# weidafeng/Efficient-SlowFast

Measured on AMD Instinct MI355X. Metric: clips/sec (8x8 224^2 SlowFast-R50+CMDA, train step fwd+bwd+allreduce+SGD), higher is better.
Workload: dtype f32

## Files before the change

### efficient-slowfast_amd/csrc/backward.hip

```cpp
#include "common.h"
#include <stdlib.h>

namespace {

constexpr int TPB = 256;


inline int pow2ceil_b(int v) {
  int p = 1;
  while (p < v) p <<= 1;
  return p;
}

template <int VEC>
__device__ __forceinline__ void bn_g(const float* __restrict__ dy, int dy_cs, int dy_coff,
                                     const float* __restrict__ y, int y_cs, int y_coff, long r, long THW, int HW,
                                     int rep, int relu, int c, float (&g)[VEC]) {
  long r0 = r;
  if (rep > 1) {
    const long n = r / THW, rem = r - n * THW;
    const long t = rem / HW, hw = rem - t * HW;
    r0 = (n * (THW / HW) * rep + t * rep) * HW + hw;
  }
#pragma unroll
  for (int e = 0; e < VEC; ++e) g[e] = 0.f;
  for (int q = 0; q < rep; ++q) {
    const float* d = dy + (r0 + (long)q * HW) * dy_cs + dy_coff + c;
    if (VEC == 4) {
      const f32x4 v = *reinterpret_cast<const f32x4*>(d);
#pragma unroll
      for (int e = 0; e < 4; ++e) g[e] += v[e];
    } else {
      g[0] += d[0];
    }
  }
  if (relu == 3) {
    if (VEC == 4) {
      const unsigned mk = reinterpret_cast<const unsigned char*>(y)[r0 * y_cs + (c >> 2)];
#pragma unroll
      for (int e = 0; e < 4; ++e)
        if (!((mk >> e) & 1u)) g[e] = 0.f;
    }
  } else if (relu) {
    const float* yp = y + r0 * y_cs + y_coff + c;
    if (VEC == 4) {
      const f32x4 v = *reinterpret_cast<const f32x4*>(yp);
#pragma unroll
      for (int e = 0; e < 4; ++e)
        if (!(v[e] > 0.f) || (relu == 2 && !(v[e] < 6.f))) g[e] = 0.f;
    } else if (!(yp[0] > 0.f) || (relu == 2 && !(yp[0] < 6.f))) {
      g[0] = 0.f;
    }
  }
}

template <int VEC>
__global__ void bn_bwd_partial_kernel(const float* __restrict__ dy, int dy_cs, int dy_coff,
                                      const float* __restrict__ y, int y_cs, int y_coff,
                                      const float* __restrict__ z, int z_cs, int z_coff, long group_rows, int chunks,
                                      int S, long THW, int HW, int C, int rep, int relu,
                                      const float* __restrict__ mean, const float* __restrict__ invstd, int CB,
                                      float* __restrict__ partial, unsigned* tickets, float* __restrict__ o1,
                                      float* __restrict__ o2, float* __restrict__ acc1, float* __restrict__ acc2) {
  __shared__ float red[2 * TPB * VEC];
  const int blk = blockIdx.x, cb = blockIdx.y;
  const int cl = threadIdx.x % CB, rl = threadIdx.x / CB, rpi = TPB / CB;
  const int c = (cb * CB + cl) * VEC;
  const int n = blk / chunks, ck = blk - n * chunks;
  const long per = (group_rows + chunks - 1) / chunks;
  const long gend = (long)(n + 1) * group_rows;
  const long r0 = (long)n * group_rows + (long)ck * per;
  const long r1 = (r0 + per < gend) ? r0 + per : gend;
  const int so = (n % S) * C;
  float s1[VEC], s2[VEC];
#pragma unroll
  for (int e = 0; e < VEC; ++e) { s1[e] = 0.f; s2[e] = 0.f; }
  if (c < C) {
    float mu[VEC], is[VEC];
#pragma unroll
    for (int e = 0; e < VEC; ++e) { mu[e] = mean[so + c + e]; is[e] = invstd[so + c + e]; }
    long r = r0 + rl;
    if constexpr (VEC == 4) if (rep == 1 && (relu == 0 || relu == 3)) {
      const unsigned char* const mk = reinterpret_cast<const unsigned char*>(y);
      for (; r + 3 * (long)rpi < r1; r += 4 * (long)rpi) {
        f32x4 gv[4], zq[4];
        unsigned mb[4];
#pragma unroll
        for (int u = 0; u < 4; ++u) {
          const long ru = r + (long)u * rpi;
          gv[u] = *reinterpret_cast<const f32x4*>(dy + ru * dy_cs + dy_coff + c);
          zq[u] = *reinterpret_cast<const f32x4*>(z + ru * z_cs + z_coff + c);
          mb[u] = relu == 3 ? mk[ru * y_cs + (c >> 2)] : 0xFu;
        }
#pragma unroll
        for (int u = 0; u < 4; ++u)
#pragma unroll
// ... 15 lines not shown
        zv[0] = z[r * z_cs + z_coff + c];
      }
#pragma unroll
      for (int e = 0; e < VEC; ++e) {
        s1[e] += g[e];
        s2[e] = fmaf(g[e], (zv[e] - mu[e]) * is[e], s2[e]);
      }
    }
  }
#pragma unroll
  for (int e = 0; e < VEC; ++e) {
    red[threadIdx.x * VEC + e] = s1[e];
    red[(TPB + threadIdx.x) * VEC + e] = s2[e];
  }
  __syncthreads();
  if (rl == 0 && c < C) {
#pragma unroll
    for (int e = 0; e < VEC; ++e) {
      float t1 = 0.f, t2 = 0.f;
      for (int i = 0; i < rpi; ++i) {
        t1 += red[(i * CB + cl) * VEC + e];
        t2 += red[(TPB + i * CB + cl) * VEC + e];
      }
      if (tickets) {
        sf_store_sc1(partial + ((long)blk * 2 + 0) * C + c + e, t1);
        sf_store_sc1(partial + ((long)blk * 2 + 1) * C + c + e, t2);
      } else {
        partial[((long)blk * 2 + 0) * C + c + e] = t1;
        partial[((long)blk * 2 + 1) * C + c + e] = t2;
      }
    }
  }
  if (!tickets) return;
  if (!sf_ticket_last(tickets + cb, gridDim.x)) return;
  const int P = gridDim.x;
  const int cbase = cb * CB * VEC;
  const int ncg = (C - cbase) < CB * VEC ? (C - cbase) : CB * VEC;
  const int q = threadIdx.x & 3;
  for (int item = threadIdx.x >> 2; item < S * ncg; item += TPB / 4) {
    const int sp = item / ncg, cc = cbase + (item - sp * ncg);
    double a1 = 0.0, a2 = 0.0;
    for (int i = q; i < P; i += 4) {
      if ((i / chunks) % S != sp) continue;
      a1 += (double)partial[((long)i * 2 + 0) * C + cc];
      a2 += (double)partial[((long)i * 2 + 1) * C + cc];
    }
    a1 += __shfl_xor(a1, 1, 64);
    a2 += __shfl_xor(a2, 1, 64);
    a1 += __shfl_xor(a1, 2, 64);
    a2 += __shfl_xor(a2, 2, 64);
    if (q == 0) {
      const int o = sp * C + cc;
      o1[o] = (float)a1;
      o2[o] = (float)a2;
      if (acc1) {
        acc1[o] += (float)a1;
        acc2[o] += (float)a2;
      }
    }
  }
}

__global__ void pair_final_kernel(const float* __restrict__ partial, int C, int P, int chunks, int S,
                                  float* __restrict__ o1, float* __restrict__ o2, float* __restrict__ acc1,
                                  float* __restrict__ acc2) {
  __shared__ double r1[64], r2[64];
  const int o = blockIdx.x;
  const int sp = o / C, c = o - sp * C;
  double s1 = 0.0, s2 = 0.0;
  int i = threadIdx.x;
  if (S == 1) {
    double a1[4] = {0.0, 0.0, 0.0, 0.0}, a2[4] = {0.0, 0.0, 0.0, 0.0};
    for (; i + 192 < P; i += 256) {
      float t1[4], t2[4];
#pragma unroll
      for (int u = 0; u < 4; ++u) {
        t1[u] = partial[((long)(i + 64 * u) * 2 + 0) * C + c];
        t2[u] = partial[((long)(i + 64 * u) * 2 + 1) * C + c];
      }
#pragma unroll
      for (int u = 0; u < 4; ++u) {
        a1[u] += (double)t1[u];
        a2[u] += (double)t2[u];
      }
    }
    s1 = (a1[0] + a1[1]) + (a1[2] + a1[3]);
    s2 = (a2[0] + a2[1]) + (a2[2] + a2[3]);
  }
  for (; i < P; i += 64) {
    if ((i / chunks) % S != sp) continue;
    s1 += (double)partial[((long)i * 2 + 0) * C + c];
    s2 += (double)partial[((long)i * 2 + 1) * C + c];
  }
// ... 257 lines not shown
  const int c = (int)(idx % C);
  const long r = idx / C;
  const float v = alpha * a[r * a_cs + a_coff + c];
  float* o = out + r * out_cs + out_coff + c;
  *o = accumulate ? *o + v : v;
}

__global__ void act_bwd_kernel(const float* __restrict__ dy, int dy_cs, int dy_coff, const float* __restrict__ y,
                               int y_cs, int y_coff, int act, float* __restrict__ dx, int dx_cs, int dx_coff, int C,
                               int accumulate, long total) {
  const long idx = (long)blockIdx.x * TPB + threadIdx.x;
  if (idx >= total) return;
  const int c = (int)(idx % C);
  const long r = idx / C;
  const float yv = y[r * y_cs + y_coff + c];
  const bool pass = (yv > 0.f) && (act != SF_ACT_RELU6 || yv < 6.f);
  const float v = pass ? dy[r * dy_cs + dy_coff + c] : 0.f;
  float* o = dx + r * dx_cs + dx_coff + c;
  *o = accumulate ? *o + v : v;
}

}

constexpr int MAX_P = 1024;
static inline void red_geometry(long rows, int C, int vec, int* CB, int* P) {
  const int cv = sf_cdiv(C, vec);
  *CB = pow2ceil_b(cv) < TPB ? pow2ceil_b(cv) : TPB;
  const int rpi = TPB / *CB;
  long p = rows / ((long)rpi * 8);
  if (p < 1) p = 1;
  if (p > MAX_P) p = MAX_P;
  *P = (int)p;
}
extern "C" long sf_bn_bwd_ws_floats(int C) { return (long)MAX_P * 2 * C; }

static int bn_bwd_reduce_launch(const float* dy, int dy_cs, int dy_coff, const float* y, int y_cs, int y_coff,
                                const float* z, int z_cs, int z_coff, int N, int T, int H, int W, int C, int S,
                                int rep, int relu, const float* mean, const float* invstd, float* dbeta,
                                float* dgamma, float* ws, void* stream, float* dbeta_acc = nullptr,
                                float* dgamma_acc = nullptr) {
  if ((dbeta_acc == nullptr) != (dgamma_acc == nullptr)) return SF_EINVAL;
  if (!dy || !z || !mean || !invstd || !dbeta || !dgamma || !ws || (relu && !y)) return SF_EINVAL;
  if (relu == 3 && (rep != 1 || (C % 4) != 0 || y_cs != C / 4 || y_coff != 0)) return SF_EINVAL;
  if (N <= 0 || T <= 0 || H <= 0 || W <= 0 || C <= 0 || rep <= 0 || S <= 0 || N % S != 0) return SF_EINVAL;
  if (S > 1 && N > MAX_P) return SF_EINVAL;
  const long rows = (long)N * T * H * W;
  const bool vec4 = (C % 4 == 0) && (dy_cs % 4 == 0) && (dy_coff % 4 == 0) && (z_cs % 4 == 0) && (z_coff % 4 == 0) &&
                    sf_aligned16(dy) && sf_aligned16(z) &&
                    (!relu || relu == 3 || ((y_cs % 4 == 0) && (y_coff % 4 == 0) && sf_aligned16(y)));
  if (relu == 3 && !vec4) return SF_EINVAL;
  const int groups = S > 1 ? N : 1;
  const long group_rows = rows / groups;
  int CB, P;
  const bool ring = sf_ticket_ring_ready((hipStream_t)stream);
  red_geometry(group_rows, C, vec4 ? 4 : 1, &CB, &P);
  const bool small = ring && S == 1 && P <= 16;
  const bool few = !small && ring && S == 1 && vec4 && C >= 256;
  const bool fused = few || small;
  const int max_p = few ? 64 : (small ? 512 : MAX_P);
  if (few && CB > 16) {
    CB = 16;
    long pp = group_rows / ((long)(TPB / CB) * 8);
    P = (int)(pp < 1 ? 1 : (pp > max_p ? max_p : pp));
  }
  if (P > max_p) P = max_p;
  if ((long)P * groups > max_p) P = max_p / groups;
  if (P < 1) return SF_EINVAL;
  const int chunks = P;
  P = chunks * groups;
  const int ncb = sf_cdiv(sf_cdiv(C, vec4 ? 4 : 1), CB);
  unsigned* tickets = fused ? sf_ticket_slots(ncb) : nullptr;
  if (fused && !tickets) return SF_ELAUNCH;
  if (vec4)
    hipLaunchKernelGGL(bn_bwd_partial_kernel<4>, dim3(P, ncb), dim3(TPB), 0, (hipStream_t)stream, dy, dy_cs, dy_coff,
                       y, y_cs, y_coff, z, z_cs, z_coff, group_rows, chunks, S, (long)T * H * W, H * W, C, rep, relu,
                       mean, invstd, CB, ws, tickets, dbeta, dgamma, dbeta_acc, dgamma_acc);
  else
    hipLaunchKernelGGL(bn_bwd_partial_kernel<1>, dim3(P, ncb), dim3(TPB), 0, (hipStream_t)stream, dy, dy_cs, dy_coff,
                       y, y_cs, y_coff, z, z_cs, z_coff, group_rows, chunks, S, (long)T * H * W, H * W, C, rep, relu,
                       mean, invstd, CB, ws, tickets, dbeta, dgamma, dbeta_acc, dgamma_acc);
  if (!fused)
    hipLaunchKernelGGL(pair_final_kernel, dim3(S * C), dim3(64), 0, (hipStream_t)stream, ws, C, P, chunks, S, dbeta,
                       dgamma, dbeta_acc, dgamma_acc);
  SF_CHECK_LAUNCH();
  return SF_OK;
}

extern "C" int sf_bn_bwd_reduce(const float* dy, int dy_cs, int dy_coff, const float* y, int y_cs, int y_coff,
                                const float* z, int z_cs, int z_coff, int N, int T, int H, int W, int C, int rep,
                                int relu, const float* mean, const float* invstd, float* dbeta, float* dgamma,
                                float* ws, void* stream) {
  return bn_bwd_reduce_launch(dy, dy_cs, dy_coff, y, y_cs, y_coff, z, z_cs, z_coff, N, T, H, W, C, 1, rep, relu, mean,
                              invstd, dbeta, dgamma, ws, stream);
}

extern "C" int sf_bn_bwd_reduce_acc(const float* dy, int dy_cs, int dy_coff, const float* y, int y_cs, int y_coff,
                                    const float* z, int z_cs, int z_coff, int N, int T, int H, int W, int C, int rep,
                                    int relu, const float* mean, const float* invstd, float* dbeta, float* dgamma,
                                    float* ws, float* dbeta_acc, float* dgamma_acc, void* stream) {
  return bn_bwd_reduce_launch(dy, dy_cs, dy_coff, y, y_cs, y_coff, z, z_cs, z_coff, N, T, H, W, C, 1, rep, relu, mean,
                              invstd, dbeta, dgamma, ws, stream, dbeta_acc, dgamma_acc);
}

extern "C" int sf_bn_bwd_reduce_split(const float* dy, int dy_cs, int dy_coff, const float* y, int y_cs, int y_coff,
                                      const float* z, int z_cs, int z_coff, int N, int T, int H, int W, int C,
                                      int nsplit, int rep, int relu, const float* mean, const float* invstd,
                                      float* dbeta, float* dgamma, float* ws, void* stream) {
  return bn_bwd_reduce_launch(dy, dy_cs, dy_coff, y, y_cs, y_coff, z, z_cs, z_coff, N, T, H, W, C, nsplit, rep, relu,
                              mean, invstd, dbeta, dgamma, ws, stream);
}

static int bn_bwd_apply_launch(const float* dy, int dy_cs, int dy_coff, const float* y, int y_cs, int y_coff,
                               const float* z, int z_cs, int z_coff, int N, int T, int H, int W, int C, int S, int rep,
                               int relu, const float* mean, const float* invstd, const float* gamma,
                               const float* dbeta, const float* dgamma, float* dz, int dz_cs, int dz_coff,
                               float* dres, int dres_cs, int dres_coff, int dres_acc, void* stream) {
// ... 589 lines not shown
```

### efficient-slowfast_amd/csrc/common.h

```cpp
#pragma once
#include <hip/hip_runtime.h>
#include <stdint.h>
#include "sfhip.h"

typedef float f32x2 __attribute__((ext_vector_type(2)));
typedef float f32x4 __attribute__((ext_vector_type(4)));
typedef float f32x16 __attribute__((ext_vector_type(16)));

#define SF_CHECK_LAUNCH()                                   \
  do {                                                      \
    if (hipPeekAtLastError() != hipSuccess) return SF_ELAUNCH; \
  } while (0)

__device__ __forceinline__ int xcd_remap(int b, int n) {
  const int q = n >> 3, r = n & 7, x = b & 7, i = b >> 3;
  return (x < r ? x * (q + 1) : r * (q + 1) + (x - r) * q) + i;
}

__device__ __forceinline__ float sf_act(float v, int act) {
  if (act == SF_ACT_RELU) return v > 0.f ? v : 0.f;
  if (act == SF_ACT_RELU6) return fminf(fmaxf(v, 0.f), 6.f);
  if (act == SF_ACT_HSIGMOID) return fminf(fmaxf(v + 3.f, 0.f), 6.f) * (1.f / 6.f);
  if (act == SF_ACT_SIGMOID) return 1.f / (1.f + __expf(-v));
  return v;
}

static inline bool sf_aligned16(const void* p) { return (reinterpret_cast<uintptr_t>(p) & 15) == 0; }
static inline int sf_cdiv(long a, long b) { return (int)((a + b - 1) / b); }

constexpr int SF_SWEEP_PARTS_MAX = 8;
int sf_sweep_parts(long units, int tiles);
int sf_attn_nw();

unsigned* sf_ticket_slots(int n);
bool sf_ticket_ring_ready(hipStream_t stream);

struct SfLdsAttr { unsigned long long done = 0; };
static inline bool sf_ensure_dyn_lds(SfLdsAttr& m, const void* fn, int bytes) {
  int dev = 0;
  if (hipGetDevice(&dev) != hipSuccess) return false;
  if (dev >= 0 && dev < 64 && ((m.done >> dev) & 1ull)) return true;
  if (hipFuncSetAttribute(fn, hipFuncAttributeMaxDynamicSharedMemorySize, bytes) != hipSuccess) return false;
  if (dev >= 0 && dev < 64) m.done |= 1ull << dev;
  return true;
}

__device__ __forceinline__ void sf_store_sc1(float* p, float v) {
  __hip_atomic_store(p, v, __ATOMIC_RELAXED, __HIP_MEMORY_SCOPE_AGENT);
}

__device__ __forceinline__ bool sf_ticket_last(unsigned* cnt, unsigned total) {
  __shared__ int s_last;
  asm volatile("s_waitcnt vmcnt(0)" ::: "memory");
  __syncthreads();
  if (threadIdx.x == 0) {
    const unsigned old = __hip_atomic_fetch_add(cnt, 1u, __ATOMIC_RELAXED, __HIP_MEMORY_SCOPE_AGENT);
    const bool last = old == total - 1u;
    if (last) {
      __hip_atomic_store(cnt, 0u, __ATOMIC_RELAXED, __HIP_MEMORY_SCOPE_AGENT);
      __builtin_amdgcn_fence(__ATOMIC_ACQUIRE, "agent");
      asm volatile("s_waitcnt vmcnt(0)" ::: "memory");
    }
    s_last = last ? 1 : 0;
  }
  __syncthreads();
  return s_last != 0;
}
```

### efficient-slowfast_amd/csrc/elementwise.hip

```cpp
#include "common.h"

namespace {

constexpr int TPB = 256;

__global__ void ncthw_to_ndhwc_kernel(const float* __restrict__ src, float* __restrict__ dst, int N, int C,
                                      int T, int H, int W, int cpad, int ph, int pw, int Hp, int Wp, long total) {
  const long idx = (long)blockIdx.x * TPB + threadIdx.x;
  if (idx >= total) return;
  const int wp = (int)(idx % Wp);
  long r = idx / Wp;
  const int hp = (int)(r % Hp);
  r /= Hp;
  const int t = (int)(r % T);
  const int n = (int)(r / T);
  const int h = hp - ph, w = wp - pw;
  const bool in = (unsigned)h < (unsigned)H && (unsigned)w < (unsigned)W;
  float* o = dst + idx * cpad;
  const long plane = (long)T * H * W;
  const float* s = src + ((long)n * C * T + t) * H * W + (long)h * W + w;
  if (cpad == 4) {
    f32x4 v = {0.f, 0.f, 0.f, 0.f};
    if (in) {
      v[0] = s[0];
// ... 336 lines not shown
}

__global__ void copy_channels_kernel(const float* __restrict__ in, int in_cs, int in_coff, float* __restrict__ out,
                                     int out_cs, int out_coff, int out_cmul, int C, long total) {
  const long idx = (long)blockIdx.x * TPB + threadIdx.x;
  if (idx >= total) return;
  const int c = (int)(idx % C);
  const long r = idx / C;
  out[r * out_cs + out_coff + (long)c * out_cmul] = in[r * in_cs + in_coff + c];
}

__global__ void channel_shuffle_kernel(const float* __restrict__ in, int in_cs, int in_coff, float* __restrict__ out,
                                       int out_cs, int out_coff, int G, int C, int accumulate, long total) {
  const long idx = (long)blockIdx.x * TPB + threadIdx.x;
  if (idx >= total) return;
  const int c = (int)(idx % C);
  const long r = idx / C;
  const float v = in[r * in_cs + in_coff + (c % G) * (C / G) + c / G];
  float* const o = out + r * out_cs + out_coff + c;
  *o = accumulate ? *o + v : v;
}


constexpr int STAT_MAX_P = 1024;

struct StatsFinal {
  double inv_rows, unbias;
  float* mean; float* var;
  const float* gamma; const float* beta;
  float eps, momentum;
  float* run_mean; float* run_var;
  float* invstd; float* scale; float* shift;
  unsigned* tickets;
};

__device__ __forceinline__ void stats_finish(const StatsFinal& f, int o, double s1, double s2, float k) {
  const double md = s1 * f.inv_rows;
  double v = s2 * f.inv_rows - md * md;
  if (v < 0.0) v = 0.0;
  const double m = md + (double)k;
  f.mean[o] = (float)m;
  f.var[o] = (float)v;
  if (f.gamma) {
    const float is = (float)(1.0 / sqrt(v + (double)f.eps));
    const float sc = f.gamma[o] * is;
    f.invstd[o] = is;
    f.scale[o] = sc;
    f.shift[o] = f.beta[o] - (float)m * sc;
    if (f.run_mean) {
      f.run_mean[o] = (1.f - f.momentum) * f.run_mean[o] + f.momentum * (float)m;
      f.run_var[o] = (1.f - f.momentum) * f.run_var[o] + f.momentum * (float)(v * f.unbias);
    }
  }
}

template <int VEC>
__global__ void stats_partial_kernel(const float* __restrict__ x, int cs, int coff, long group_rows, int chunks,
                                     int S, int C, int CB, float* __restrict__ partial, const StatsFinal fin) {
  __shared__ float red[2 * TPB * VEC];
  const int blk = blockIdx.x, cb = blockIdx.y;
  const int cl = threadIdx.x % CB, rl = threadIdx.x / CB, rpi = TPB / CB;
  const int c = (cb * CB + cl) * VEC;
  const int n = blk / chunks, ck = blk - n * chunks;
  const long per = (group_rows + chunks - 1) / chunks;
  const long gend = (long)(n + 1) * group_rows;
  const long r0 = (long)n * group_rows + (long)ck * per;
  const long r1 = (r0 + per < gend) ? r0 + per : gend;
  const long krow = (long)(n % S) * group_rows;
  float s1[VEC], s2[VEC], k[VEC];
#pragma unroll
  for (int e = 0; e < VEC; ++e) { s1[e] = 0.f; s2[e] = 0.f; k[e] = 0.f; }
  if (c < C) {
#pragma unroll
    for (int e = 0; e < VEC; ++e) k[e] = x[krow * cs + coff + c + e];
    long r = r0 + rl;
    if constexpr (VEC == 4) {
      for (; r + 3 * (long)rpi < r1; r += 4 * (long)rpi) {
        f32x4 v[4];
#pragma unroll
        for (int u = 0; u < 4; ++u) v[u] = *reinterpret_cast<const f32x4*>(x + (r + (long)u * rpi) * cs + coff + c);
#pragma unroll
        for (int u = 0; u < 4; ++u)
#pragma unroll
          for (int e = 0; e < 4; ++e) {
            const float d = v[u][e] - k[e];
            s1[e] += d;
            s2[e] = fmaf(d, d, s2[e]);
          }
// ... 9 lines not shown
          s2[e] = fmaf(d, d, s2[e]);
        }
      } else {
        const float d = x[r * cs + coff + c] - k[0];
        s1[0] += d;
        s2[0] = fmaf(d, d, s2[0]);
      }
    }
  }
#pragma unroll
  for (int e = 0; e < VEC; ++e) {
    red[threadIdx.x * VEC + e] = s1[e];
    red[(TPB + threadIdx.x) * VEC + e] = s2[e];
  }
  __syncthreads();
  if (rl == 0 && c < C) {
#pragma unroll
    for (int e = 0; e < VEC; ++e) {
      float t1 = 0.f, t2 = 0.f;
      for (int i = 0; i < rpi; ++i) {
        t1 += red[(i * CB + cl) * VEC + e];
        t2 += red[(TPB + i * CB + cl) * VEC + e];
      }
      if (fin.tickets) {
        sf_store_sc1(partial + ((long)blk * 2 + 0) * C + c + e, t1);
        sf_store_sc1(partial + ((long)blk * 2 + 1) * C + c + e, t2);
      } else {
        partial[((long)blk * 2 + 0) * C + c + e] = t1;
        partial[((long)blk * 2 + 1) * C + c + e] = t2;
      }
    }
  }
  if (!fin.tickets) return;
  if (!sf_ticket_last(fin.tickets + cb, gridDim.x)) return;
  const int P = gridDim.x;
  const int cbase = cb * CB * VEC;
  const int ncg = (C - cbase) < CB * VEC ? (C - cbase) : CB * VEC;
  const int q = threadIdx.x & 3;
  for (int item = threadIdx.x >> 2; item < S * ncg; item += TPB / 4) {
    const int sp = item / ncg, cc = cbase + (item - sp * ncg);
    double s1 = 0.0, s2 = 0.0;
    for (int i = q; i < P; i += 4) {
      if ((i / chunks) % S != sp) continue;
      s1 += (double)partial[((long)i * 2 + 0) * C + cc];
      s2 += (double)partial[((long)i * 2 + 1) * C + cc];
    }
    s1 += __shfl_xor(s1, 1, 64);
    s2 += __shfl_xor(s2, 1, 64);
    s1 += __shfl_xor(s1, 2, 64);
    s2 += __shfl_xor(s2, 2, 64);
    if (q == 0) stats_finish(fin, sp * C + cc, s1, s2, x[(long)sp * group_rows * cs + coff + cc]);
  }
}

__global__ void stats_final_kernel(const float* __restrict__ x, int cs, int coff, long group_rows, int chunks, int S,
                                   const float* __restrict__ partial, int C, int P, double inv_rows, double unbias,
                                   float* __restrict__ mean, float* __restrict__ var,
                                   const float* __restrict__ gamma, const float* __restrict__ beta, float eps,
                                   float momentum, float* __restrict__ run_mean, float* __restrict__ run_var,
                                   float* __restrict__ invstd, float* __restrict__ scale, float* __restrict__ shift) {
  __shared__ double r1[64], r2[64];
  const int o = blockIdx.x;
  const int sp = o / C, c = o - sp * C;
  double s1 = 0.0, s2 = 0.0;
  int i = threadIdx.x;
  if (S == 1) {
    double a1[4] = {0.0, 0.0, 0.0, 0.0}, a2[4] = {0.0, 0.0, 0.0, 0.0};
    for (; i + 192 < P; i += 256) {
      float t1[4], t2[4];
#pragma unroll
      for (int u = 0; u < 4; ++u) {
        t1[u] = partial[((long)(i + 64 * u) * 2 + 0) * C + c];
        t2[u] = partial[((long)(i + 64 * u) * 2 + 1) * C + c];
      }
#pragma unroll
      for (int u = 0; u < 4; ++u) {
        a1[u] += (double)t1[u];
        a2[u] += (double)t2[u];
      }
    }
    s1 = (a1[0] + a1[1]) + (a1[2] + a1[3]);
    s2 = (a2[0] + a2[1]) + (a2[2] + a2[3]);
  }
  for (; i < P; i += 64) {
    if ((i / chunks) % S != sp) continue;
// ... 200 lines not shown
    __syncthreads();
    if (co < (unsigned)it.Cout && c0 + lx < (unsigned)it.cin_pad)
      for (unsigned tap = 0; tap < taps; ++tap)
        it.wp[((long)co * taps + tap) * it.cin_pad + c0 + lx] = seg[ly * pitch + lx * taps + tap];
    return;
  }
  const unsigned Q = (unsigned)it.Cin * (unsigned)it.taps;
  const unsigned tq = (Q + 31u) / 32u;
  const unsigned t = b - nbw;
  const unsigned tco = t / tq, tqi = t - tco * tq;
  const unsigned q0 = tqi * 32u, co0 = tco * 32u;
  const unsigned lx = threadIdx.x & 31u, ly = threadIdx.x >> 5;
#pragma unroll
  for (int k = 0; k < 4; ++k) {
    const unsigned co = co0 + ly + 8u * k, q = q0 + lx;
    tile[ly + 8 * k][lx] = (co < (unsigned)it.Cout && q < Q) ? it.w[(long)co * Q + q] : 0.f;
  }
  __syncthreads();
#pragma unroll
  for (int k = 0; k < 4; ++k) {
    const unsigned q = q0 + ly + 8u * k, co = co0 + lx;
    if (q < Q && co < (unsigned)it.cout_pad) it.wtp[(long)q * it.cout_pad + co] = tile[lx][ly + 8 * k];
  }
}

inline int pow2ceil(int v) {
  int p = 1;
  while (p < v) p <<= 1;
  return p;
}

}

#include <atomic>
namespace {
constexpr int TICKET_RING = 1 << 16, TICKET_MAXDEV = 16;
unsigned* g_ticket_ring[TICKET_MAXDEV] = {};
std::atomic<unsigned> g_ticket_next[TICKET_MAXDEV];
}

bool sf_ticket_ring_ready(hipStream_t stream) {
  int dev = 0;
  if (hipGetDevice(&dev) != hipSuccess || dev < 0 || dev >= TICKET_MAXDEV) return false;
  if (g_ticket_ring[dev]) return true;
  hipStreamCaptureStatus st = hipStreamCaptureStatusNone;
  if (hipStreamIsCapturing(stream, &st) != hipSuccess || st != hipStreamCaptureStatusNone) return false;
  unsigned* p = nullptr;
  if (hipMalloc(&p, TICKET_RING * sizeof(unsigned)) != hipSuccess) return false;
  if (hipMemset(p, 0, TICKET_RING * sizeof(unsigned)) != hipSuccess) return false;
  g_ticket_ring[dev] = p;
  return true;
}

unsigned* sf_ticket_slots(int n) {
  int dev = 0;
  if (hipGetDevice(&dev) != hipSuccess || dev < 0 || dev >= TICKET_MAXDEV || n <= 0 || n > 4096) return nullptr;
  if (!g_ticket_ring[dev]) return nullptr;
  const unsigned take = ((unsigned)n + 63u) & ~63u;
  unsigned off;
  do {
    off = g_ticket_next[dev].fetch_add(take) % TICKET_RING;
  } while (off + take > (unsigned)TICKET_RING);
  return g_ticket_ring[dev] + off;
}

extern "C" int sf_abi_version(void) { return 1; }
extern "C" const char* sf_build_arch(void) { return "gfx950"; }

extern "C" int sf_ncthw_to_ndhwc(const float* src, float* dst, int N, int C, int T, int H, int W, int cpad,
                                 int ph, int pw, int Wp, void* stream) {
  if (!src || !dst || N <= 0 || C <= 0 || T <= 0 || H <= 0 || W <= 0 || cpad < C || ph < 0 || pw < 0 ||
      Wp < W + 2 * pw)
    return SF_EINVAL;
  if (cpad == 4 && !sf_aligned16(dst)) return SF_EALIGN;
  const int Hp = H + 2 * ph;
  const long total = (long)N * T * Hp * Wp;
  hipLaunchKernelGGL(ncthw_to_ndhwc_kernel, dim3(sf_cdiv(total, TPB)), dim3(TPB), 0, (hipStream_t)stream, src,
                     dst, N, C, T, H, W, cpad, ph, pw, Hp, Wp, total);
  SF_CHECK_LAUNCH();
  return SF_OK;
}

extern "C" int sf_ndhwc_to_ncthw(const float* src, int cs, int coff, float* dst, int N, int C, int T, int H,
                                 int W, void* stream) {
  if (!src || !dst || N <= 0 || C <= 0 || T <= 0 || H <= 0 || W <= 0 || cs < coff + C) return SF_EINVAL;
  const long thw = (long)T * H * W;
  const long total = (long)N * C * thw;
  hipLaunchKernelGGL(ndhwc_to_ncthw_kernel, dim3(sf_cdiv(total, TPB)), dim3(TPB), 0, (hipStream_t)stream, src,
                     cs, coff, dst, C, thw, total);
  SF_CHECK_LAUNCH();
  return SF_OK;
}

extern "C" int sf_pool_fwd(const sf_pool_desc* d, const float* in, float* out, void* stream) {
  if (!d || !in || !out || d->C <= 0 || d->kT <= 0 || d->kH <= 0 || d->kW <= 0) return SF_EINVAL;
  if (d->N <= 0 || d->To <= 0 || d->Ho <= 0 || d->Wo <= 0) return SF_EINVAL;
// ... 78 lines not shown
  hipLaunchKernelGGL(tmax_partial_kernel, dim3(POOL_P, ncb, N), dim3(TPB), 0, (hipStream_t)stream, x, cs, coff, T,
                     H * W, C, alpha, CB, ws);
  const float inv = 1.f / (float)((long)(T / alpha) * H * W);
  hipLaunchKernelGGL(tmax_final_kernel, dim3(sf_cdiv(C, TPB), N), dim3(TPB), 0, (hipStream_t)stream, ws, C, inv,
                     pooled);
  SF_CHECK_LAUNCH();
  return SF_OK;
}

extern "C" int sf_gate_apply(const float* x, int cs, int coff, int N, int T, int H, int W, int C, int alpha,
                             const float* pooled, const float* w3, const float* scale, const float* bias, int act,
                             float* out, int out_cs, int out_coff, void* stream) {
  if (!x || !pooled || !out || N <= 0 || C <= 0 || alpha <= 0 || (T % alpha) != 0) return SF_EINVAL;
  if ((scale == nullptr) != (bias == nullptr)) return SF_EINVAL;
  if (act != SF_ACT_NONE && act != SF_ACT_RELU) return SF_EINVAL;
  const bool vec4 = (C % 4 == 0) && (cs % 4 == 0) && (coff % 4 == 0) && (out_cs % 4 == 0) && (out_coff % 4 == 0) &&
                    sf_aligned16(x) && sf_aligned16(out);
  const long rows = (long)(T / alpha) * H * W;
  const long total = rows * (vec4 ? C / 4 : C);
  int gx = sf_cdiv(total, TPB);
  if (gx > 2048) gx = 2048;
  const size_t shm = (size_t)C * sizeof(float);
  if (vec4)
    hipLaunchKernelGGL(gate_apply_kernel<4>, dim3(gx, N), dim3(TPB), shm, (hipStream_t)stream, x, cs, coff, T,
                       H * W, C, alpha, pooled, w3, scale, bias, act, out, out_cs, out_coff);
  else
    hipLaunchKernelGGL(gate_apply_kernel<1>, dim3(gx, N), dim3(TPB), shm, (hipStream_t)stream, x, cs, coff, T,
                       H * W, C, alpha, pooled, w3, scale, bias, act, out, out_cs, out_coff);
  SF_CHECK_LAUNCH();
  return SF_OK;
}


extern "C" long sf_channel_stats_ws_floats(int C) { return (long)STAT_MAX_P * 2 * C; }

static int stats_launch(const float* x, int cs, int coff, int groups, long group_rows, int S, int C, float* mean,
                        float* var, float* ws, const float* gamma, const float* beta, float eps, float momentum,
                        float* run_mean, float* run_var, float* invstd, float* scale, float* shift, hipStream_t s) {
  if (groups > STAT_MAX_P || S <= 0 || groups % S != 0) return SF_EINVAL;
  const bool vec4 = (C % 4 == 0) && (cs % 4 == 0) && (coff % 4 == 0) && sf_aligned16(x);
  const int cv = sf_cdiv(C, vec4 ? 4 : 1);
  const bool ring = sf_ticket_ring_ready(s);
  const int CB = pow2ceil(cv) < TPB ? pow2ceil(cv) : TPB;
  const bool fused = ring && S == 1 && groups == 1 && group_rows / ((long)(TPB / CB) * 8) <= 16;
  const int rpi = TPB / CB;
  const int max_p = fused ? 512 : STAT_MAX_P;
  if (groups > max_p) return SF_EINVAL;
  long ch = group_rows / ((long)rpi * 8);
  if (ch < 1) ch = 1;
  if (ch * groups > max_p) ch = max_p / groups;
  const int chunks = (int)ch, P = chunks * groups;
  const long srows = group_rows * (groups / S);
  const int ncb = sf_cdiv(cv, CB);
  StatsFinal fin;
  fin.inv_rows = 1.0 / (double)srows;
  fin.unbias = srows > 1 ? (double)srows / (double)(srows - 1) : 1.0;
  fin.mean = mean; fin.var = var; fin.gamma = gamma; fin.beta = beta; fin.eps = eps; fin.momentum = momentum;
  fin.run_mean = run_mean; fin.run_var = run_var; fin.invstd = invstd; fin.scale = scale; fin.shift = shift;
  fin.tickets = fused ? sf_ticket_slots(ncb) : nullptr;
  if (fused && !fin.tickets) return SF_ELAUNCH;
  if (vec4)
    hipLaunchKernelGGL(stats_partial_kernel<4>, dim3(P, ncb), dim3(TPB), 0, s, x, cs, coff, group_rows, chunks, S, C, CB,
                       ws, fin);
  else
    hipLaunchKernelGGL(stats_partial_kernel<1>, dim3(P, ncb), dim3(TPB), 0, s, x, cs, coff, group_rows, chunks, S, C, CB,
                       ws, fin);
  if (!fused)
    hipLaunchKernelGGL(stats_final_kernel, dim3(S * C), dim3(64), 0, s, x, cs, coff, group_rows, chunks, S, ws, C, P,
                       fin.inv_rows, fin.unbias, mean, var, gamma, beta, eps, momentum, run_mean, run_var, invstd, scale,
                       shift);
  SF_CHECK_LAUNCH();
  return SF_OK;
}

__global__ void stats_merge_kernel(const float* __restrict__ parts, int P, int C, const StatsFinal f) {
  __shared__ double red[16][9];
  const int quad = blockIdx.x, nq = C >> 2;
  const int tid = threadIdx.x, lane = tid & 63, wave = tid >> 6, nwave = blockDim.x >> 6;
  const f32x4 R = *reinterpret_cast<const f32x4*>(parts + (long)quad * 16 + 4);
  double n = 0.0, s1[4] = {0.0, 0.0, 0.0, 0.0}, s2[4] = {0.0, 0.0, 0.0, 0.0};
  auto add = [&](const f32x4& cnt, const f32x4& k, const f32x4& a1, const f32x4& a2) {
    const double ni = (double)cnt[0];
    n += ni;
#pragma unroll
    for (int e = 0; e < 4; ++e) {
      const double dk = (double)k[e] - (double)R[e], t1 = (double)a1[e];
      s1[e] += t1 + ni * dk;
      s2[e] += (double)a2[e] + dk * (2.0 * t1 + ni * dk);
    }
  };
  const int step = blockDim.x;
  int i = tid;
  for (; i + 3 * step < P; i += 4 * step) {
    f32x4 v[4][4];
#pragma unroll
    for (int u = 0; u < 4; ++u) {
      const float* q = parts + ((long)(i + u * step) * nq + quad) * 16;
#pragma unroll
      for (int w = 0; w < 4; ++w) v[u][w] = *reinterpret_cast<const f32x4*>(q + 4 * w);
    }
#pragma unroll
    for (int u = 0; u < 4; ++u) add(v[u][0], v[u][1], v[u][2], v[u][3]);
  }
// ... 8 lines not shown
#pragma unroll
    for (int e = 0; e < 4; ++e) {
      s1[e] += __shfl_xor(s1[e], off, 64);
      s2[e] += __shfl_xor(s2[e], off, 64);
    }
  }
  if (lane == 0) {
    red[wave][0] = n;
#pragma unroll
    for (int e = 0; e < 4; ++e) { red[wave][1 + e] = s1[e]; red[wave][5 + e] = s2[e]; }
  }
  __syncthreads();
  if (tid < 4) {
    double N = 0.0, t1 = 0.0, t2 = 0.0;
    for (int w = 0; w < nwave; ++w) { N += red[w][0]; t1 += red[w][1 + tid]; t2 += red[w][5 + tid]; }
    StatsFinal g = f;
    g.inv_rows = 1.0 / N;
    g.unbias = N > 1.0 ? N / (N - 1.0) : 1.0;
    stats_finish(g, quad * 4 + tid, t1, t2, R[tid]);
  }
}

extern "C" int sf_bn_train_stats_merge(const float* parts, int P, int C, const float* gamma, const float* beta, float eps,
                                       float momentum, float* run_mean, float* run_var, float* mean, float* var,
                                       float* invstd, float* scale, float* shift, void* stream) {
  if (!parts || P <= 0 || C <= 0 || (C % 4) != 0 || !gamma || !beta || !mean || !var || !invstd || !scale || !shift)
    return SF_EINVAL;
  if ((run_mean == nullptr) != (run_var == nullptr) || !sf_aligned16(parts)) return SF_EINVAL;
  StatsFinal fin;
  fin.inv_rows = 1.0; fin.unbias = 1.0;
  fin.mean = mean; fin.var = var; fin.gamma = gamma; fin.beta = beta; fin.eps = eps; fin.momentum = momentum;
  fin.run_mean = run_mean; fin.run_var = run_var; fin.invstd = invstd; fin.scale = scale; fin.shift = shift;
  fin.tickets = nullptr;
  hipLaunchKernelGGL(stats_merge_kernel, dim3(C / 4), dim3(P > 1024 ? 1024 : 256), 0, (hipStream_t)stream, parts, P, C,
                     fin);
  SF_CHECK_LAUNCH();
  return SF_OK;
}

extern "C" int sf_channel_stats(const float* x, int cs, int coff, long rows, int C, float* mean, float* var,
                                float* ws, void* stream) {
  if (!x || !mean || !var || !ws || rows <= 0 || C <= 0) return SF_EINVAL;
  return stats_launch(x, cs, coff, 1, rows, 1, C, mean, var, ws, nullptr, nullptr, 0.f, 0.f, nullptr, nullptr, nullptr,
                      nullptr, nullptr, (hipStream_t)stream);
}

extern "C" int sf_bn_train_stats(const float* x, int cs, int coff, long rows, int C, const float* gamma,
                                 const float* beta, float eps, float momentum, float* run_mean, float* run_var,
                                 float* mean, float* var, float* invstd, float* scale, float* shift, float* ws,
                                 void* stream) {
  if (!x || !gamma || !beta || !mean || !var || !invstd || !scale || !shift || !ws || rows <= 0 || C <= 0)
    return SF_EINVAL;
  if ((run_mean == nullptr) != (run_var == nullptr)) return SF_EINVAL;
  return stats_launch(x, cs, coff, 1, rows, 1, C, mean, var, ws, gamma, beta, eps, momentum, run_mean, run_var,
                      invstd, scale, shift, (hipStream_t)stream);
}

extern "C" int sf_bn_train_stats_split(const float* x, int cs, int coff, int N, long rows_per_sample, int C,
                                       int nsplit, const float* gamma, const float* beta, float eps, float momentum,
                                       float* run_mean, float* run_var, float* mean, float* var, float* invstd,
                                       float* scale, float* shift, float* ws, void* stream) {
  if (!x || !gamma || !beta || !mean || !var || !invstd || !scale || !shift || !ws || N <= 0 ||
      rows_per_sample <= 0 || C <= 0 || nsplit <= 0 || N % nsplit != 0)
    return SF_EINVAL;
  if ((run_mean == nullptr) != (run_var == nullptr)) return SF_EINVAL;
  return stats_launch(x, cs, coff, N, rows_per_sample, nsplit, C, mean, var, ws, gamma, beta, eps, momentum, run_mean,
// ... 124 lines not shown
```

Measured before the change: 150.8.

## Use two-level ticketed fold for BN stats and backward channel reductions

For single-group BatchNorm forward stats and backward dbeta/dgamma reductions, the final cross-block reduction now runs in two levels. Groups of 32 partial blocks are summed by the last-arriving block of each group into a double-precision L2 workspace, and the globally last block folds those group sums. New geometry caps channels per block at 64 so more column blocks and row chunks run in parallel. The ticket allocator is also reworked to work under stream capture, so the fused path is always available, with a fallback final kernel when no ticket slots are granted. This drops the separate final kernel launch and the serial single-block reduction over up to 1024 partials, at the cost of extra atomics, workspace and more complex allocation.

New measurement: 150.5. No clear change (-0.2%).

```diff
diff --git a/efficient-slowfast_amd/csrc/backward.hip b/efficient-slowfast_amd/csrc/backward.hip
--- a/efficient-slowfast_amd/csrc/backward.hip
+++ b/efficient-slowfast_amd/csrc/backward.hip
@@ -54,14 +54,27 @@
   }
 }
 
+struct PairFin {
+  float* o1; float* o2; float* acc1; float* acc2;
+  __device__ void operator()(int c, double s1, double s2) const {
+    o1[c] = (float)s1;
+    o2[c] = (float)s2;
+    if (acc1) {
+      acc1[c] += (float)s1;
+      acc2[c] += (float)s2;
+    }
+  }
+};
+
 template <int VEC>
 __global__ void bn_bwd_partial_kernel(const float* __restrict__ dy, int dy_cs, int dy_coff,
                                       const float* __restrict__ y, int y_cs, int y_coff,
                                       const float* __restrict__ z, int z_cs, int z_coff, long group_rows, int chunks,
                                       int S, long THW, int HW, int C, int rep, int relu,
                                       const float* __restrict__ mean, const float* __restrict__ invstd, int CB,
-                                      float* __restrict__ partial, unsigned* tickets, float* __restrict__ o1,
-                                      float* __restrict__ o2, float* __restrict__ acc1, float* __restrict__ acc2) {
+                                      float* __restrict__ partial, double* l2, unsigned* tickets,
+                                      float* __restrict__ o1, float* __restrict__ o2, float* __restrict__ acc1,
+                                      float* __restrict__ acc2) {
   __shared__ float red[2 * TPB * VEC];
   const int blk = blockIdx.x, cb = blockIdx.y;
   const int cl = threadIdx.x % CB, rl = threadIdx.x / CB, rpi = TPB / CB;
@@ -143,33 +156,11 @@
     }
   }
   if (!tickets) return;
-  if (!sf_ticket_last(tickets + cb, gridDim.x)) return;
   const int P = gridDim.x;
   const int cbase = cb * CB * VEC;
   const int ncg = (C - cbase) < CB * VEC ? (C - cbase) : CB * VEC;
-  const int q = threadIdx.x & 3;
-  for (int item = threadIdx.x >> 2; item < S * ncg; item += TPB / 4) {
-    const int sp = item / ncg, cc = cbase + (item - sp * ncg);
-    double a1 = 0.0, a2 = 0.0;
-    for (int i = q; i < P; i += 4) {
-      if ((i / chunks) % S != sp) continue;
-      a1 += (double)partial[((long)i * 2 + 0) * C + cc];
-      a2 += (double)partial[((long)i * 2 + 1) * C + cc];
-    }
-    a1 += __shfl_xor(a1, 1, 64);
-    a2 += __shfl_xor(a2, 1, 64);
-    a1 += __shfl_xor(a1, 2, 64);
-    a2 += __shfl_xor(a2, 2, 64);
-    if (q == 0) {
-      const int o = sp * C + cc;
-      o1[o] = (float)a1;
-      o2[o] = (float)a2;
-      if (acc1) {
-        acc1[o] += (float)a1;
-        acc2[o] += (float)a2;
-      }
-    }
-  }
+  sf_fold_finish(partial, l2, tickets + cb * (1 + sf_fold_groups(P)), blk, P, C, cbase, ncg,
+                 PairFin{o1, o2, acc1, acc2});
 }
 
 __global__ void pair_final_kernel(const float* __restrict__ partial, int C, int P, int chunks, int S,
@@ -493,7 +484,10 @@
   if (p > MAX_P) p = MAX_P;
   *P = (int)p;
 }
-extern "C" long sf_bn_bwd_ws_floats(int C) { return (long)MAX_P * 2 * C; }
+extern "C" long sf_bn_bwd_ws_floats(int C) { return (long)MAX_P * 2 * C + 2 + sf_fold_l2_floats(C); }
+static inline double* bwd_ws_l2(float* ws, int C) {
+  return reinterpret_cast<double*>((reinterpret_cast<uintptr_t>(ws + (long)MAX_P * 2 * C) + 7) & ~(uintptr_t)7);
+}
 
 static int bn_bwd_reduce_launch(const float* dy, int dy_cs, int dy_coff, const float* y, int y_cs, int y_coff,
                                 const float* z, int z_cs, int z_coff, int N, int T, int H, int W, int C, int S,
@@ -513,36 +507,43 @@
   const int groups = S > 1 ? N : 1;
   const long group_rows = rows / groups;
   int CB, P;
-  const bool ring = sf_ticket_ring_ready((hipStream_t)stream);
+  if (S == 1) {
+    const int vec = vec4 ? 4 : 1;
+    sf_fold_geometry(rows, sf_cdiv(C, vec), vec, &CB, &P);
+    const int ncb = sf_cdiv(sf_cdiv(C, vec), CB);
+    double* l2 = bwd_ws_l2(ws, C);
+    const long nslots = (long)ncb * (1 + sf_fold_groups(P));
+    unsigned* tickets = nslots <= 4096 ? sf_ticket_slots((int)nslots, (hipStream_t)stream) : nullptr;
+    if (vec4)
+      hipLaunchKernelGGL(bn_bwd_partial_kernel<4>, dim3(P, ncb), dim3(TPB), 0, (hipStream_t)stream, dy, dy_cs, dy_coff,
+                         y, y_cs, y_coff, z, z_cs, z_coff, rows, P, 1, (long)T * H * W, H * W, C, rep, relu, mean, invstd,
+                         CB, ws, l2, tickets, dbeta, dgamma, dbeta_acc, dgamma_acc);
+    else
+      hipLaunchKernelGGL(bn_bwd_partial_kernel<1>, dim3(P, ncb), dim3(TPB), 0, (hipStream_t)stream, dy, dy_cs, dy_coff,
+                         y, y_cs, y_coff, z, z_cs, z_coff, rows, P, 1, (long)T * H * W, H * W, C, rep, relu, mean, invstd,
+                         CB, ws, l2, tickets, dbeta, dgamma, dbeta_acc, dgamma_acc);
+    if (!tickets)
+      hipLaunchKernelGGL(sf_fold_final_kernel<PairFin>, dim3(ncb), dim3(TPB), 0, (hipStream_t)stream, ws, l2, P, C,
+                         CB * vec, PairFin{dbeta, dgamma, dbeta_acc, dgamma_acc});
+    SF_CHECK_LAUNCH();
+    return SF_OK;
+  }
   red_geometry(group_rows, C, vec4 ? 4 : 1, &CB, &P);
-  const bool small = ring && S == 1 && P <= 16;
-  const bool few = !small && ring && S == 1 && vec4 && C >= 256;
-  const bool fused = few || small;
-  const int max_p = few ? 64 : (small ? 512 : MAX_P);
-  if (few && CB > 16) {
-    CB = 16;
-    long pp = group_rows / ((long)(TPB / CB) * 8);
-    P = (int)(pp < 1 ? 1 : (pp > max_p ? max_p : pp));
-  }
-  if (P > max_p) P = max_p;
-  if ((long)P * groups > max_p) P = max_p / groups;
+  if ((long)P * groups > MAX_P) P = MAX_P / groups;
   if (P < 1) return SF_EINVAL;
   const int chunks = P;
   P = chunks * groups;
   const int ncb = sf_cdiv(sf_cdiv(C, vec4 ? 4 : 1), CB);
-  unsigned* tickets = fused ? sf_ticket_slots(ncb) : nullptr;
-  if (fused && !tickets) return SF_ELAUNCH;
   if (vec4)
     hipLaunchKernelGGL(bn_bwd_partial_kernel<4>, dim3(P, ncb), dim3(TPB), 0, (hipStream_t)stream, dy, dy_cs, dy_coff,
                        y, y_cs, y_coff, z, z_cs, z_coff, group_rows, chunks, S, (long)T * H * W, H * W, C, rep, relu,
-                       mean, invstd, CB, ws, tickets, dbeta, dgamma, dbeta_acc, dgamma_acc);
+                       mean, invstd, CB, ws, nullptr, nullptr, dbeta, dgamma, dbeta_acc, dgamma_acc);
   else
     hipLaunchKernelGGL(bn_bwd_partial_kernel<1>, dim3(P, ncb), dim3(TPB), 0, (hipStream_t)stream, dy, dy_cs, dy_coff,
                        y, y_cs, y_coff, z, z_cs, z_coff, group_rows, chunks, S, (long)T * H * W, H * W, C, rep, relu,
-                       mean, invstd, CB, ws, tickets, dbeta, dgamma, dbeta_acc, dgamma_acc);
-  if (!fused)
-    hipLaunchKernelGGL(pair_final_kernel, dim3(S * C), dim3(64), 0, (hipStream_t)stream, ws, C, P, chunks, S, dbeta,
-                       dgamma, dbeta_acc, dgamma_acc);
+                       mean, invstd, CB, ws, nullptr, nullptr, dbeta, dgamma, dbeta_acc, dgamma_acc);
+  hipLaunchKernelGGL(pair_final_kernel, dim3(S * C), dim3(64), 0, (hipStream_t)stream, ws, C, P, chunks, S, dbeta,
+                     dgamma, dbeta_acc, dgamma_acc);
   SF_CHECK_LAUNCH();
   return SF_OK;
 }
diff --git a/efficient-slowfast_amd/csrc/common.h b/efficient-slowfast_amd/csrc/common.h
--- a/efficient-slowfast_amd/csrc/common.h
+++ b/efficient-slowfast_amd/csrc/common.h
@@ -32,8 +32,7 @@
 int sf_sweep_parts(long units, int tiles);
 int sf_attn_nw();
 
-unsigned* sf_ticket_slots(int n);
-bool sf_ticket_ring_ready(hipStream_t stream);
+unsigned* sf_ticket_slots(int n, hipStream_t stream);
 
 struct SfLdsAttr { unsigned long long done = 0; };
 static inline bool sf_ensure_dyn_lds(SfLdsAttr& m, const void* fn, int bytes) {
@@ -66,3 +65,106 @@
   __syncthreads();
   return s_last != 0;
 }
+
+__device__ __forceinline__ void sf_store_sc1(double* p, double v) {
+  __hip_atomic_store(p, v, __ATOMIC_RELAXED, __HIP_MEMORY_SCOPE_AGENT);
+}
+
+constexpr int SF_FOLD_G = 32;
+constexpr int SF_FOLD_MAX_P = SF_FOLD_G * SF_FOLD_G;
+constexpr int SF_FOLD_MAX_CH = 64;
+__host__ __device__ static inline int sf_fold_groups(int P) { return (P + SF_FOLD_G - 1) / SF_FOLD_G; }
+static inline long sf_fold_l2_floats(int C) { return (long)SF_FOLD_G * 2 * C * 2; }
+
+static inline void sf_fold_geometry(long rows, int cv, int vec, int* CB, int* P) {
+  int cb = 1;
+  while (cb < cv && cb * vec < SF_FOLD_MAX_CH) cb <<= 1;
+  const int ncb = (cv + cb - 1) / cb;
+  long pmax = 1024 / ncb;
+  if (pmax < 16) pmax = 16;
+  if (pmax > SF_FOLD_MAX_P) pmax = SF_FOLD_MAX_P;
+  long p = rows / ((long)(256 / cb) * 8);
+  if (p < 1) p = 1;
+  if (p > pmax) p = pmax;
+  *CB = cb;
+  *P = (int)p;
+}
+
+template <typename T>
+__device__ __forceinline__ void sf_fold_lanes(const T* p, long plane, long stride, int cnt, int q, int L, double& a1,
+                                              double& a2) {
+  constexpr int J = SF_FOLD_G / 4;
+  T t1[J], t2[J];
+#pragma unroll
+  for (int j = 0; j < J; ++j) {
+    const int i = q + j * L;
+    const bool ok = i < cnt;
+    t1[j] = ok ? p[(long)i * stride] : (T)0;
+    t2[j] = ok ? p[(long)i * stride + plane] : (T)0;
+  }
+  a1 = 0.0;
+  a2 = 0.0;
+#pragma unroll
+  for (int j = 0; j < J; ++j) {
+    a1 += (double)t1[j];
+    a2 += (double)t2[j];
+  }
+  for (int off = 1; off < L; off <<= 1) {
+    a1 += __shfl_xor(a1, off, 64);
+    a2 += __shfl_xor(a2, off, 64);
+  }
+}
+
+template <class Fin>
+__device__ __forceinline__ void sf_fold_finish(const float* partial, double* l2, unsigned* tk, int blk, int P, int C,
+                                               int cbase, int nch, Fin fin) {
+  const int ng = (P + SF_FOLD_G - 1) / SF_FOLD_G, g = blk / SF_FOLD_G;
+  const int gcnt = (P - g * SF_FOLD_G) < SF_FOLD_G ? (P - g * SF_FOLD_G) : SF_FOLD_G;
+  if (!sf_ticket_last(tk + 1 + g, (unsigned)gcnt)) return;
+  int L = SF_FOLD_G;
+  while (L * nch > 256) L >>= 1;
+  const int ch = (int)threadIdx.x / L, q = (int)threadIdx.x % L;
+  const bool live = ch < nch;
+  const int c = cbase + (live ? ch : 0);
+  double a1, a2;
+  sf_fold_lanes<float>(partial + (long)g * SF_FOLD_G * 2 * C + c, C, 2L * C, live ? gcnt : 0, q, L, a1, a2);
+  if (ng == 1) {
+    if (live && q == 0) fin(c, a1, a2);
+    return;
+  }
+  if (live && q == 0) {
+    sf_store_sc1(l2 + ((long)g * 2 + 0) * C + c, a1);
+    sf_store_sc1(l2 + ((long)g * 2 + 1) * C + c, a2);
+  }
+  if (!sf_ticket_last(tk, (unsigned)ng)) return;
+  sf_fold_lanes<double>(l2 + c, C, 2L * C, live ? ng : 0, q, L, a1, a2);
+  if (live && q == 0) fin(c, a1, a2);
+}
+
+template <class Fin>
+__global__ __launch_bounds__(256) void sf_fold_final_kernel(const float* __restrict__ partial, double* l2, int P, int C,
+                                                            int chw, const Fin fin) {
+  const int cbase = blockIdx.x * chw;
+  const int nch = (C - cbase) < chw ? (C - cbase) : chw;
+  const int ng = (P + SF_FOLD_G - 1) / SF_FOLD_G;
+  int L = SF_FOLD_G;
+  while (L * nch > 256) L >>= 1;
+  const int ch = (int)threadIdx.x / L, q = (int)threadIdx.x % L;
+  const bool live = ch < nch;
+  const int c = cbase + (live ? ch : 0);
+  double a1 = 0.0, a2 = 0.0;
+  for (int g = 0; g < ng; ++g) {
+    const int gcnt = (P - g * SF_FOLD_G) < SF_FOLD_G ? (P - g * SF_FOLD_G) : SF_FOLD_G;
+    sf_fold_lanes<float>(partial + (long)g * SF_FOLD_G * 2 * C + c, C, 2L * C, live ? gcnt : 0, q, L, a1, a2);
+    if (ng > 1 && live && q == 0) {
+      l2[((long)g * 2 + 0) * C + c] = a1;
+      l2[((long)g * 2 + 1) * C + c] = a2;
+    }
+  }
+  if (ng > 1) {
+    __threadfence_block();
+    __syncthreads();
+    sf_fold_lanes<double>(l2 + c, C, 2L * C, live ? ng : 0, q, L, a1, a2);
+  }
+  if (live && q == 0) fin(c, a1, a2);
+}
diff --git a/efficient-slowfast_amd/csrc/elementwise.hip b/efficient-slowfast_amd/csrc/elementwise.hip
--- a/efficient-slowfast_amd/csrc/elementwise.hip
+++ b/efficient-slowfast_amd/csrc/elementwise.hip
@@ -392,6 +392,7 @@
   float* run_mean; float* run_var;
   float* invstd; float* scale; float* shift;
   unsigned* tickets;
+  double* l2;
 };
 
 __device__ __forceinline__ void stats_finish(const StatsFinal& f, int o, double s1, double s2, float k) {
@@ -414,6 +415,12 @@
   }
 }
 
+struct StatsFin {
+  StatsFinal f;
+  const float* xk;
+  __device__ void operator()(int c, double s1, double s2) const { stats_finish(f, c, s1, s2, xk[c]); }
+};
+
 template <int VEC>
 __global__ void stats_partial_kernel(const float* __restrict__ x, int cs, int coff, long group_rows, int chunks,
                                      int S, int C, int CB, float* __restrict__ partial, const StatsFinal fin) {
@@ -489,25 +496,11 @@
     }
   }
   if (!fin.tickets) return;
-  if (!sf_ticket_last(fin.tickets + cb, gridDim.x)) return;
   const int P = gridDim.x;
   const int cbase = cb * CB * VEC;
   const int ncg = (C - cbase) < CB * VEC ? (C - cbase) : CB * VEC;
-  const int q = threadIdx.x & 3;
-  for (int item = threadIdx.x >> 2; item < S * ncg; item += TPB / 4) {
-    const int sp = item / ncg, cc = cbase + (item - sp * ncg);
-    double s1 = 0.0, s2 = 0.0;
-    for (int i = q; i < P; i += 4) {
-      if ((i / chunks) % S != sp) continue;
-      s1 += (double)partial[((long)i * 2 + 0) * C + cc];
-      s2 += (double)partial[((long)i * 2 + 1) * C + cc];
-    }
-    s1 += __shfl_xor(s1, 1, 64);
-    s2 += __shfl_xor(s2, 1, 64);
-    s1 += __shfl_xor(s1, 2, 64);
-    s2 += __shfl_xor(s2, 2, 64);
-    if (q == 0) stats_finish(fin, sp * C + cc, s1, s2, x[(long)sp * group_rows * cs + coff + cc]);
-  }
+  sf_fold_finish(partial, fin.l2, fin.tickets + cb * (1 + sf_fold_groups(P)), blk, P, C, cbase, ncg,
+                 StatsFin{fin, x + coff});
 }
 
 __global__ void stats_final_kernel(const float* __restrict__ x, int cs, int coff, long group_rows, int chunks, int S,
@@ -774,36 +767,47 @@
 
 }
 
-#include <atomic>
+#include <mutex>
 namespace {
-constexpr int TICKET_RING = 1 << 16, TICKET_MAXDEV = 16;
+constexpr unsigned TICKET_EAGER = 1u << 17, TICKET_RING = 1u << 18, TICKET_LINE = 64;
+constexpr int TICKET_MAXDEV = 16;
+std::mutex g_ticket_mu;
 unsigned* g_ticket_ring[TICKET_MAXDEV] = {};
-std::atomic<unsigned> g_ticket_next[TICKET_MAXDEV];
-}
-
-bool sf_ticket_ring_ready(hipStream_t stream) {
-  int dev = 0;
-  if (hipGetDevice(&dev) != hipSuccess || dev < 0 || dev >= TICKET_MAXDEV) return false;
-  if (g_ticket_ring[dev]) return true;
-  hipStreamCaptureStatus st = hipStreamCaptureStatusNone;
-  if (hipStreamIsCapturing(stream, &st) != hipSuccess || st != hipStreamCaptureStatusNone) return false;
-  unsigned* p = nullptr;
-  if (hipMalloc(&p, TICKET_RING * sizeof(unsigned)) != hipSuccess) return false;
-  if (hipMemset(p, 0, TICKET_RING * sizeof(unsigned)) != hipSuccess) return false;
-  g_ticket_ring[dev] = p;
-  return true;
-}
-
-unsigned* sf_ticket_slots(int n) {
+unsigned g_ticket_eager[TICKET_MAXDEV] = {};
+unsigned g_ticket_cap[TICKET_MAXDEV] = {};
+}
+
+unsigned* sf_ticket_slots(int n, hipStream_t stream) {
   int dev = 0;
   if (hipGetDevice(&dev) != hipSuccess || dev < 0 || dev >= TICKET_MAXDEV || n <= 0 || n > 4096) return nullptr;
-  if (!g_ticket_ring[dev]) return nullptr;
-  const unsigned take = ((unsigned)n + 63u) & ~63u;
-  unsigned off;
-  do {
-    off = g_ticket_next[dev].fetch_add(take) % TICKET_RING;
-  } while (off + take > (unsigned)TICKET_RING);
-  return g_ticket_ring[dev] + off;
+  hipStreamCaptureStatus st = hipStreamCaptureStatusNone;
+  if (hipStreamIsCapturing(stream, &st) != hipSuccess) return nullptr;
+  const bool capturing = st != hipStreamCaptureStatusNone;
+  std::lock_guard<std::mutex> lock(g_ticket_mu);
+  if (!g_ticket_ring[dev]) {
+    if (capturing) return nullptr;
+    unsigned* p = nullptr;
+    if (hipMalloc(&p, TICKET_RING * sizeof(unsigned)) != hipSuccess) return nullptr;
+    if (hipMemset(p, 0, TICKET_RING * sizeof(unsigned)) != hipSuccess || hipDeviceSynchronize() != hipSuccess) {
+      (void)hipFree(p);
+      return nullptr;
+    }
+    g_ticket_ring[dev] = p;
+  }
+  const unsigned take = ((unsigned)n + TICKET_LINE - 1u) & ~(TICKET_LINE - 1u);
+  if (capturing) {
+    if (g_ticket_cap[dev] + take > TICKET_RING - TICKET_EAGER) return nullptr;
+    unsigned* r = g_ticket_ring[dev] + TICKET_EAGER + g_ticket_cap[dev];
+    g_ticket_cap[dev] += take;
+    return r;
+  }
+  if (g_ticket_eager[dev] + take > TICKET_EAGER) {
+    if (hipDeviceSynchronize() != hipSuccess) return nullptr;
+    g_ticket_eager[dev] = 0;
+  }
+  unsigned* r = g_ticket_ring[dev] + g_ticket_eager[dev];
+  g_ticket_eager[dev] += take;
+  return r;
 }
 
 extern "C" int sf_abi_version(void) { return 1; }
@@ -948,7 +952,10 @@
 }
 
 
-extern "C" long sf_channel_stats_ws_floats(int C) { return (long)STAT_MAX_P * 2 * C; }
+extern "C" long sf_channel_stats_ws_floats(int C) { return (long)STAT_MAX_P * 2 * C + 2 + sf_fold_l2_floats(C); }
+static inline double* stat_ws_l2(float* ws, int C) {
+  return reinterpret_cast<double*>((reinterpret_cast<uintptr_t>(ws + (long)STAT_MAX_P * 2 * C) + 7) & ~(uintptr_t)7);
+}
 
 static int stats_launch(const float* x, int cs, int coff, int groups, long group_rows, int S, int C, float* mean,
                         float* var, float* ws, const float* gamma, const float* beta, float eps, float momentum,
@@ -956,35 +963,50 @@
   if (groups > STAT_MAX_P || S <= 0 || groups % S != 0) return SF_EINVAL;
   const bool vec4 = (C % 4 == 0) && (cs % 4 == 0) && (coff % 4 == 0) && sf_aligned16(x);
   const int cv = sf_cdiv(C, vec4 ? 4 : 1);
-  const bool ring = sf_ticket_ring_ready(s);
+  StatsFinal fin;
+  fin.mean = mean; fin.var = var; fin.gamma = gamma; fin.beta = beta; fin.eps = eps; fin.momentum = momentum;
+  fin.run_mean = run_mean; fin.run_var = run_var; fin.invstd = invstd; fin.scale = scale; fin.shift = shift;
+  fin.tickets = nullptr;
+  fin.l2 = stat_ws_l2(ws, C);
+  if (S == 1 && groups == 1) {
+    int CB, P;
+    sf_fold_geometry(group_rows, cv, vec4 ? 4 : 1, &CB, &P);
+    const int ncb = sf_cdiv(cv, CB);
+    fin.inv_rows = 1.0 / (double)group_rows;
+    fin.unbias = group_rows > 1 ? (double)group_rows / (double)(group_rows - 1) : 1.0;
+    const long nslots = (long)ncb * (1 + sf_fold_groups(P));
+    fin.tickets = nslots <= 4096 ? sf_ticket_slots((int)nslots, s) : nullptr;
+    if (vec4)
+      hipLaunchKernelGGL(stats_partial_kernel<4>, dim3(P, ncb), dim3(TPB), 0, s, x, cs, coff, group_rows, P, 1, C, CB, ws,
+                         fin);
+    else
+      hipLaunchKernelGGL(stats_partial_kernel<1>, dim3(P, ncb), dim3(TPB), 0, s, x, cs, coff, group_rows, P, 1, C, CB, ws,
+                         fin);
+    if (!fin.tickets)
+      hipLaunchKernelGGL(sf_fold_final_kernel<StatsFin>, dim3(ncb), dim3(TPB), 0, s, ws, fin.l2, P, C,
+                         CB * (vec4 ? 4 : 1), StatsFin{fin, x + coff});
+    SF_CHECK_LAUNCH();
+    return SF_OK;
+  }
   const int CB = pow2ceil(cv) < TPB ? pow2ceil(cv) : TPB;
-  const bool fused = ring && S == 1 && groups == 1 && group_rows / ((long)(TPB / CB) * 8) <= 16;
   const int rpi = TPB / CB;
-  const int max_p = fused ? 512 : STAT_MAX_P;
-  if (groups > max_p) return SF_EINVAL;
   long ch = group_rows / ((long)rpi * 8);
   if (ch < 1) ch = 1;
-  if (ch * groups > max_p) ch = max_p / groups;
+  if (ch * groups > STAT_MAX_P) ch = STAT_MAX_P / groups;
   const int chunks = (int)ch, P = chunks * groups;
   const long srows = group_rows * (groups / S);
   const int ncb = sf_cdiv(cv, CB);
-  StatsFinal fin;
   fin.inv_rows = 1.0 / (double)srows;
   fin.unbias = srows > 1 ? (double)srows / (double)(srows - 1) : 1.0;
-  fin.mean = mean; fin.var = var; fin.gamma = gamma; fin.beta = beta; fin.eps = eps; fin.momentum = momentum;
-  fin.run_mean = run_mean; fin.run_var = run_var; fin.invstd = invstd; fin.scale = scale; fin.shift = shift;
-  fin.tickets = fused ? sf_ticket_slots(ncb) : nullptr;
-  if (fused && !fin.tickets) return SF_ELAUNCH;
   if (vec4)
     hipLaunchKernelGGL(stats_partial_kernel<4>, dim3(P, ncb), dim3(TPB), 0, s, x, cs, coff, group_rows, chunks, S, C, CB,
                        ws, fin);
   else
     hipLaunchKernelGGL(stats_partial_kernel<1>, dim3(P, ncb), dim3(TPB), 0, s, x, cs, coff, group_rows, chunks, S, C, CB,
                        ws, fin);
-  if (!fused)
-    hipLaunchKernelGGL(stats_final_kernel, dim3(S * C), dim3(64), 0, s, x, cs, coff, group_rows, chunks, S, ws, C, P,
-                       fin.inv_rows, fin.unbias, mean, var, gamma, beta, eps, momentum, run_mean, run_var, invstd, scale,
-                       shift);
+  hipLaunchKernelGGL(stats_final_kernel, dim3(S * C), dim3(64), 0, s, x, cs, coff, group_rows, chunks, S, ws, C, P,
+                     fin.inv_rows, fin.unbias, mean, var, gamma, beta, eps, momentum, run_mean, run_var, invstd, scale,
+                     shift);
   SF_CHECK_LAUNCH();
   return SF_OK;
 }
@@ -1059,6 +1081,7 @@
   fin.mean = mean; fin.var = var; fin.gamma = gamma; fin.beta = beta; fin.eps = eps; fin.momentum = momentum;
   fin.run_mean = run_mean; fin.run_var = run_var; fin.invstd = invstd; fin.scale = scale; fin.shift = shift;
   fin.tickets = nullptr;
+  fin.l2 = nullptr;
   hipLaunchKernelGGL(stats_merge_kernel, dim3(C / 4), dim3(P > 1024 ? 1024 : 256), 0, (hipStream_t)stream, parts, P, C,
                      fin);
   SF_CHECK_LAUNCH();
```
